# rajasekarv/vega

Measured on AMD Instinct MI355X. Metric: rows/sec (whole node) reduce_by_key i64→i64, 1e9 rows, 1/2/4/8 GPU, higher is better.
Workload: dtype int64; 1 GPU; C1: 1e9 (i64,i64) uniform keys in [0,2^63), reduce_by_key(sum), 256 partitions (BASELINE.json configs[1]); weak scaling: --rows per GPU; rows_per_gpu=1000000000, key_bits=63, nparts=256, distinct_keys_out=1000000000

## Files before the change

vega_amd/csrc/vega_kernels.hip:

```cpp

#include <hip/hip_runtime.h>
#include <cmath>
#include <cstdint>
#include <cstdio>
#include <cstring>
#include <mutex>
#include <string>
#include <unordered_map>
#include <vector>

#include "../../include/vega_common.h"
#include "vega_internal.h"

#define HIP_TRY(x)                                                              \
    do {                                                                        \
        hipError_t _e = (x);                                                    \
        if (_e != hipSuccess) return _e;                                        \
    } while (0)

namespace vega {

constexpr int BLOCK = 256;
constexpr int IPT = 16;
constexpr int TILE = BLOCK * IPT;
// ... 1324 lines not shown
        uint64_t g0;
        int m;
        bounds(tile, &g0, &m);
        const int a0 = (int)(t0 - g0), a1 = (int)(t1 - g0);
        if (threadIdx.x == 0) s_bad = 0;
#pragma unroll
        for (int q = 0; q < FIN_LPT; ++q) {
            int li = q * FIN_B + threadIdx.x;
            h[q] = (uint32_t)vega_hash_u64(r[q].x);
            if (li < m) s_row[li] = r[q];
            if (lane == 63) s_edge[q * (FIN_B / 64) + w] = h[q] >> 8;
        }
        __syncthreads();
        VEGA_PHASE_MARK(0)
        const uint32_t next = tile + gridDim.x;
        if (next < ntiles) fetch(next);
        const bool done = order_tile(g0, m, a0, a1);
        if (done) {
            const int lo = lo_out;
            uint32_t heads = 0;
            uint16_t si[FIN_FT / FIN_B], sp[FIN_FT / FIN_B];
#pragma unroll
            for (int q = 0; q < FIN_FT / FIN_B; ++q) {
                const int p = a0 + q * FIN_B + threadIdx.x;
                const int pc = p < a1 ? p : a1 - 1;
                si[q] = s_src[pc];
                sp[q] = s_src[pc > lo ? pc - 1 : pc];
            }
            ulonglong2 row[FIN_FT / FIN_B];
            uint64_t pkey[FIN_FT / FIN_B];
#pragma unroll
            for (int q = 0; q < FIN_FT / FIN_B; ++q) {
                row[q] = s_row[si[q]];
                pkey[q] = s_row[sp[q]].x;
            }
#pragma unroll
            for (int q = 0; q < FIN_FT / FIN_B; ++q) {
                const int p = a0 + q * FIN_B + threadIdx.x;
                if (p < a1) ((ulonglong2 *)out)[g0 + p] = row[q];
                const bool head = p < a1 && (p == lo || row[q].x != pkey[q]);
                heads += (uint32_t)__popcll(__ballot(head));
            }
            if (lane == 0) s_heads[w] = heads;
        }
        VEGA_PHASE_MARK(4)
        __syncthreads();
        if (done && threadIdx.x == 0) {
            uint32_t t = 0;
#pragma unroll
            for (int i = 0; i < FIN_B / 64; ++i) t += s_heads[i];
            fin_heads[tile] = t;
        }
        VEGA_PHASE_MARK(5)
        tile = next;
    }
    if (PROF && lane == 0)
        for (int i = 0; i < FIN_PHASES; ++i) atomicAdd(&phc[FIN_PHASE0 + i], pacc[i]);
#undef VEGA_PHASE_MARK
}

__global__ void k_unpack_rows(const uint64_t *pk, uint64_t n, uint64_t *k, uint64_t *v) {
    uint64_t stride = (uint64_t)gridDim.x * blockDim.x;
    for (uint64_t i = (uint64_t)blockIdx.x * blockDim.x + threadIdx.x; i < n; i += stride) {
        ulonglong2 r = ((const ulonglong2 *)pk)[i];
        k[i] = r.x;
        v[i] = r.y;
    }
}

hipError_t group_sort_u64(hipStream_t s, const uint64_t *in_k, const uint64_t *in_v,
                          uint64_t n, int force_hbytes, int *order_tag,
                          int want_packed, int *out_packed, Ws &ws,
                          const uint64_t **res_k, const uint64_t **res_v,
                          int route, int *route_taken, const uint32_t **fin_heads) {
    *res_k = in_k;
    *res_v = in_v;
    if (out_packed) *out_packed = 0;
    if (order_tag) *order_tag = 0;
    if (route_taken) *route_taken = 0;
    if (fin_heads) *fin_heads = nullptr;
    if (n <= 1) return hipSuccess;
    if (n >= (1ULL << 32)) return hipErrorNotSupported;
    uint32_t nb = nblocks_for(n);

    uint64_t *pA = (uint64_t *)ws.take(n * 16);
    uint64_t *pB = (uint64_t *)ws.take(n * 16);
    unsigned long long *desc = (unsigned long long *)ws.take((size_t)256 * nb * 8);
    uint32_t *gbase_d = (uint32_t *)ws.take(8 * 256 * 4);
    uint32_t *ticket = (uint32_t *)ws.take(256);
    uint32_t *h8 = (uint32_t *)ws.take(8 * 256 * 4);
    int *d_err = (int *)ws.take(256);
    int *d_abort = (int *)ws.take(256);
    unsigned long long *ff_d = (unsigned long long *)ws.take(
        ((size_t)((nb + OSW_GRP - 1) / OSW_GRP) +
         (size_t)((nb + OSW_SUP - 1) / OSW_SUP)) * 256 * 8);
    uint32_t *h32buf = (uint32_t *)ws.take(n * 4);
    unsigned long long *wl = (unsigned long long *)ws.take(CLEANUP_WL_CAP * 8);
    uint32_t *wl_count = (uint32_t *)ws.take(256);
    uint32_t *fh_d = (uint32_t *)ws.take(((size_t)2 * nb + 1) * 4);
    if (!pA || !pB || !desc || !gbase_d || !ticket || !h8 || !d_err || !d_abort ||
        !ff_d || !h32buf || !wl || !wl_count || !fh_d)
        return hipErrorOutOfMemory;
    HIP_TRY(hipMemsetAsync(d_abort, 0, 4, s));
    HIP_TRY(hipMemsetAsync(desc, 0, (size_t)nb * 256 * 8, s));
    int ptag_ctr = 0;
    const int strict = (force_hbytes != 0 || order_tag != nullptr) ? 1 : 0;

    static thread_local uint32_t hh[8 * 256];
    static thread_local uint32_t gb_host[8 * 256];
    bool pass_on[8] = {true, true, true, true, true, true, true, true};

    auto exact_hists = [&](bool hashsrc, int nbl, int *active) -> hipError_t {
        HIP_TRY(hipMemsetAsync(h8, 0, 8 * 256 * 4, s));
        {
            ProfScope ps(hashsrc ? "ghist" : "hist8", s);
            uint32_t gb = nb < 2048 ? nb : 2048;
            if (hashsrc && nbl == 4)
                hipLaunchKernelGGL((k_hist8t<true, 4>), dim3(gb), dim3(BLOCK), 0, s, in_k, n, h8);
            else if (hashsrc)
                hipLaunchKernelGGL((k_hist8t<true, 5>), dim3(gb), dim3(BLOCK), 0, s, in_k, n, h8);
            else
                hipLaunchKernelGGL((k_hist8t<false, 8>), dim3(gb), dim3(BLOCK), 0, s, in_k, n, h8);
            HIP_TRY(hipGetLastError());
        }
        HIP_TRY(hipMemcpyAsync(hh, h8, 8 * 256 * 4, hipMemcpyDeviceToHost, s));
        HIP_TRY(hipStreamSynchronize(s));
        *active = 0;
        for (int p = 0; p < 8; ++p) {
            int nz = 0;
            uint32_t running = 0;
            for (int d = 0; d < 256; ++d) {
                nz += hh[p * 256 + d] != 0;
                gb_host[p * 256 + d] = running;
                running += hh[p * 256 + d];
            }
            pass_on[p] = nz > 1;
            *active += pass_on[p];
        }
        return hipMemcpyAsync(gbase_d, gb_host, 8 * 256 * 4, hipMemcpyHostToDevice, s);
    };

    auto run_key_passes = [&](const uint64_t **rk, const uint64_t **rv) -> hipError_t {
        int plist[8], np = 0;
        for (int p = 0; p < 8; ++p)
            if (pass_on[p]) plist[np++] = p;
        if (np == 0) { *rk = in_k; *rv = in_v; return hipSuccess; }
        const uint64_t *cur = nullptr;
        for (int i = 0; i < np; ++i) {
            int p = plist[i];
            bool in_pk = i > 0, out_pk = i < np - 1;
            uint64_t *dbuf = ((i & 1) == 0) ? pA : pB;
            uint64_t *dk = dbuf;
            uint64_t *dv = out_pk ? nullptr : dbuf + n;
            RadixDigit df{8 * p};
            HIP_TRY(scatter_pass_osw(s, i == 0 ? in_k : cur, i == 0 ? in_v : nullptr,
                                     n, gbase_d + p * 256, desc, ticket,
                                     dk, dv, nullptr, d_abort, ff_d, ptag_ctr++, true, in_pk, out_pk, df, "radix_scatter"));
            cur = dk;
        }
        *rk = cur;
        *rv = cur + n;
        return hipSuccess;
    };

    int a_est = 8;
    bool samp_repeat = false;
    double bucket_rows = 0;
    HIP_TRY(sample_active_passes(s, in_k, n, ws, &a_est, &samp_repeat, &bucket_rows));

    const uint64_t *cur_k = in_k, *cur_v = in_v;
    if (a_est <= 5 && route == 0) {
        int active = 8;
        HIP_TRY(exact_hists(false, 8, &active));
        if (active <= 5) {
            HIP_TRY(run_key_passes(res_k, res_v));
            int ab = 0;
            HIP_TRY(hipMemcpyAsync(&ab, d_abort, 4, hipMemcpyDeviceToHost, s));
            HIP_TRY(hipStreamSynchronize(s));
            return ab ? hipErrorUnknown : hipSuccess;
        }
    }

    const int hbytes = force_hbytes ? force_hbytes : ((n <= (1ULL << 30)) ? 4 : 5);
    int active5 = 0;
    HIP_TRY(exact_hists(true, hbytes, &active5));
    const bool keep_pk = want_packed != 0;
    if (!strict && hbytes == 4 && keep_pk && route != 1 &&
        (route == 2 || (!samp_repeat && bucket_rows >= FIN_MIN_BUCKET_ROWS))) {
        for (int i = 1; i < 4; ++i) {
            uint64_t *dk = (i & 1) ? pA : pB;
            HashByteDigit df{8 * i};
            HIP_TRY(scatter_pass_osw(s, i == 1 ? in_k : cur_k, i == 1 ? in_v : nullptr,
                                     n, gbase_d + i * 256, desc, ticket, dk, nullptr, nullptr,
                                     d_abort, ff_d, ptag_ctr++, true, i > 1, true, df, "radix_scatter"));
            cur_k = dk;
        }
        HIP_TRY(hipMemsetAsync(d_err, 0, 4, s));
        {
            ProfScope ps("group_cleanup", s);
            ProfScope pk("bucket_finish", s);
            const uint32_t ntiles = (uint32_t)((n + FIN_FT - 1) / FIN_FT);
            unsigned long long *phc = phase_prof_buf();
            const dim3 grid(ntiles < FIN_GRID ? ntiles : FIN_GRID);
            if (phc)
                hipLaunchKernelGGL(k_bucket_finish<true>, grid, dim3(FIN_B), 0, s, cur_k, pB, n,
                                   d_err, fh_d, phc);
            else
                hipLaunchKernelGGL(k_bucket_finish<false>, grid, dim3(FIN_B), 0, s, cur_k, pB, n,
                                   d_err, fh_d, nullptr);
            HIP_TRY(hipGetLastError());
        }
        int fl[2] = {0, 0};
        HIP_TRY(hipMemcpyAsync(&fl[0], d_err, 4, hipMemcpyDeviceToHost, s));
        HIP_TRY(hipMemcpyAsync(&fl[1], d_abort, 4, hipMemcpyDeviceToHost, s));
        HIP_TRY(hipStreamSynchronize(s));
        if (fl[1]) return hipErrorUnknown;
        if (!fl[0]) {
            if (out_packed) *out_packed = 1;
            if (route_taken) *route_taken = 2;
            if (fin_heads) *fin_heads = fh_d;
            *res_k = pB;
            *res_v = nullptr;
            return hipSuccess;
        }
        cur_k = in_k;
        cur_v = in_v;
    }
    if (route_taken) *route_taken = 1;
    for (int i = 0; i < hbytes; ++i) {
        bool in_pk = i > 0, out_pk = keep_pk || (i < hbytes - 1);
        bool last = i == hbytes - 1;
        uint64_t *dbuf = ((i & 1) == 0) ? pA : pB;
        uint64_t *dk = dbuf;
        uint64_t *dv = out_pk ? nullptr : dbuf + n;
        HashByteDigit df{8 * i};
        HIP_TRY(scatter_pass_osw(s, i == 0 ? in_k : cur_k, i == 0 ? in_v : nullptr,
                                 n, gbase_d + i * 256, desc, ticket,
                                 dk, dv, last ? h32buf : nullptr,
                                 d_abort, ff_d, ptag_ctr++, true, in_pk, out_pk, df, "radix_scatter"));
        cur_k = dk;
        cur_v = out_pk ? nullptr : dk + n;
    }
    HIP_TRY(hipMemsetAsync(d_err, 0, 4, s));
    HIP_TRY(hipMemsetAsync(wl_count, 0, 4, s));
    {
        ProfScope ps("group_cleanup", s);
        uint32_t gb = nb < 2048 ? nb : 2048;
        hipLaunchKernelGGL(k_group_cleanup, dim3(gb), dim3(BLOCK), 0, s,
                           (uint64_t *)cur_k, (uint64_t *)cur_v, h32buf, n,
                           keep_pk ? 1 : 0, strict, d_err, wl, wl_count);
        HIP_TRY(hipGetLastError());
        hipLaunchKernelGGL(k_group_cleanup_long, dim3(512), dim3(BLOCK), 0, s,
                           cur_k, h32buf, n, keep_pk ? 1 : 0, strict, d_err, wl, wl_count);
        HIP_TRY(hipGetLastError());
    }
    int flags[2] = {0, 0};
    HIP_TRY(hipMemcpyAsync(&flags[0], d_err, 4, hipMemcpyDeviceToHost, s));
    HIP_TRY(hipMemcpyAsync(&flags[1], d_abort, 4, hipMemcpyDeviceToHost, s));
    HIP_TRY(hipStreamSynchronize(s));
    if (flags[1]) return hipErrorUnknown;
    int err = flags[0];
    if (err) {
        int active = 8;
        HIP_TRY(exact_hists(false, 8, &active));
        HIP_TRY(run_key_passes(&cur_k, &cur_v));
        int ab2 = 0;
        HIP_TRY(hipMemcpyAsync(&ab2, d_abort, 4, hipMemcpyDeviceToHost, s));
        HIP_TRY(hipStreamSynchronize(s));
        if (ab2) return hipErrorUnknown;
    } else if (keep_pk && out_packed) {
        *out_packed = 1;
    }
    if (order_tag && !err) *order_tag = (hbytes == 4) ? 4 : 0;
    *res_k = cur_k;
    *res_v = cur_v;
    return hipSuccess;
}


template <bool PK>
__global__ void k_head_count(const uint64_t *k, uint64_t n, uint32_t *hc) {
    __shared__ uint32_t wsum[BLOCK / 64];
    uint64_t tbase = (uint64_t)blockIdx.x * TILE;
    uint32_t c = 0;
#pragma unroll
    for (int j = 0; j < IPT; ++j) {
        uint64_t idx = tbase + (uint64_t)j * BLOCK + threadIdx.x;
        if (idx < n)
            c += (idx == 0) || (k[PK ? 2 * idx : idx] != k[PK ? 2 * (idx - 1) : idx - 1]);
    }
    for (int off = 32; off > 0; off >>= 1) c += __shfl_down(c, off);
    int lane = threadIdx.x & 63, w = threadIdx.x >> 6;
    if (lane == 0) wsum[w] = c;
    __syncthreads();
    if (threadIdx.x == 0) {
        uint32_t t = 0;
        for (int i = 0; i < BLOCK / 64; ++i) t += wsum[i];
        hc[blockIdx.x] = t;
    }
}

#define SEG_B 512
#define SEG_IPT 8
template <int OP, bool PK>
__global__ __launch_bounds__(SEG_B) void k_seg_emit(
    const uint64_t *__restrict__ k, const void *__restrict__ vv, uint64_t n,
    const uint32_t *__restrict__ head_base, uint32_t hstride,
    int64_t *__restrict__ out_k, void *__restrict__ out_vv,
    uint32_t *__restrict__ lead_seg, double *__restrict__ lead_part) {
    __shared__ uint32_t wsc[SEG_B / 64];
    constexpr bool NEED_V = (OP != 1);

    const int t = threadIdx.x, lane = t & 63, w = t >> 6;
    const uint64_t tbase = (uint64_t)blockIdx.x * TILE;
    const uint64_t *v = (const uint64_t *)vv;
    const uint64_t c0g = tbase + (uint64_t)t * SEG_IPT;

    uint64_t kk[SEG_IPT], sv[SEG_IPT];
    if (c0g + SEG_IPT <= n) {
        if (PK) {
            const ulonglong2 *rp = reinterpret_cast<const ulonglong2 *>(k) + c0g;
#pragma unroll
            for (int j = 0; j < SEG_IPT; ++j) {
                ulonglong2 r2 = rp[j];
                kk[j] = r2.x;
                sv[j] = r2.y;
            }
        } else {
            const ulonglong2 *kp = reinterpret_cast<const ulonglong2 *>(k + c0g);
            const ulonglong2 *vp = reinterpret_cast<const ulonglong2 *>(v + c0g);
#pragma unroll
            for (int j2 = 0; j2 < SEG_IPT / 2; ++j2) {
                ulonglong2 t2 = kp[j2];
                kk[2 * j2] = t2.x;
                kk[2 * j2 + 1] = t2.y;
                if (NEED_V) {
                    ulonglong2 u2 = vp[j2];
                    sv[2 * j2] = u2.x;
                    sv[2 * j2 + 1] = u2.y;
                }
            }
        }
    } else {
#pragma unroll
        for (int j = 0; j < SEG_IPT; ++j) {
            uint64_t gi = c0g + j;
            kk[j] = (gi < n) ? k[PK ? 2 * gi : gi] : ~0ULL;
            if (NEED_V || PK) sv[j] = (gi < n) ? (PK ? k[2 * gi + 1] : v[gi]) : 0;
        }
    }
    uint64_t prev = (c0g > 0 && c0g <= n) ? k[PK ? 2 * (c0g - 1) : c0g - 1] : 0;

    uint32_t cnt = 0;
#pragma unroll
    for (int j = 0; j < SEG_IPT; ++j) {
        uint64_t gi = c0g + j;
        if (gi < n) {
            uint64_t pk = (j > 0) ? kk[j - 1] : prev;
            cnt += (gi == 0) || (kk[j] != pk);
        }
    }
    uint32_t inc = cnt;
    for (int off = 1; off < 64; off <<= 1) {
        uint32_t u = __shfl_up(inc, off);
        if (lane >= off) inc += u;
    }
    if (lane == 63) wsc[w] = inc;
    __syncthreads();
    uint32_t excl = inc - cnt;
    for (int i = 0; i < w; ++i) excl += wsc[i];

    if (OP == 2) {
        uint64_t chunk_id = (uint64_t)blockIdx.x * SEG_B + t;
        int64_t sid = (int64_t)head_base[(size_t)blockIdx.x * hstride] + excl - 1;
        if (c0g >= n) {
            lead_seg[chunk_id] = 0xFFFFFFFFu;
            return;
        }
        int nvalid = (int)((n - c0g < SEG_IPT) ? (n - c0g) : SEG_IPT);
        int fh = -1;
        for (int j = 0; j < nvalid; ++j) {
            uint64_t pk2 = (j > 0) ? kk[j - 1] : prev;
            if (c0g + j == 0 || kk[j] != pk2) { fh = j; break; }
        }
        int le = (fh >= 0) ? fh : nvalid;
        if (le > 0) {
            double lead = 0.0;
            for (int j = 0; j < le; ++j) lead += __longlong_as_double((long long)sv[j]);
            lead_seg[chunk_id] = (uint32_t)sid;
            lead_part[chunk_id] = lead;
        } else {
            lead_seg[chunk_id] = 0xFFFFFFFFu;
        }
        if (fh >= 0) {
            double acc = 0.0;
            for (int j = fh; j < nvalid; ++j) {
                uint64_t pk2 = (j > 0) ? kk[j - 1] : prev;
                bool head = (c0g + j == 0) || (kk[j] != pk2);
                if (head) {
                    if (j > fh) ((double *)out_vv)[sid] = acc;
                    sid++;
                    out_k[sid] = (int64_t)kk[j];
                    acc = 0.0;
                }
                acc += __longlong_as_double((long long)sv[j]);
            }
            ((double *)out_vv)[sid] = acc;
        }
        return;
    }

    const uint64_t chunk_id = (uint64_t)blockIdx.x * SEG_B + t;
    if (c0g >= n) {
        lead_seg[chunk_id] = 0xFFFFFFFFu;
        return;
    }
    constexpr int64_t IDENT = (OP == 3) ? INT64_MAX : (OP == 4) ? INT64_MIN : 0;
    auto fold = [](int64_t a, uint64_t x) -> int64_t {
        if (OP == 0) return (int64_t)((uint64_t)a + x);
        if (OP == 1) return a + 1;
        if (OP == 3) return (int64_t)x < a ? (int64_t)x : a;
        return (int64_t)x > a ? (int64_t)x : a;
    };
    int64_t segid = (int64_t)head_base[(size_t)blockIdx.x * hstride] + excl - 1;
    if (cnt == SEG_IPT && c0g + SEG_IPT <= n) {
        int64_t s0 = segid + 1;
        int64_t *okp = (int64_t *)out_k + s0;
        uint64_t *ovp = (uint64_t *)out_vv + s0;
        if ((s0 & 1) == 0) {
            ulonglong2 *ok2 = (ulonglong2 *)okp;
            ulonglong2 *ov2 = (ulonglong2 *)ovp;
#pragma unroll
            for (int j = 0; j < SEG_IPT / 2; ++j) {
                ok2[j] = make_ulonglong2(kk[2 * j], kk[2 * j + 1]);
                if (OP == 1) ov2[j] = make_ulonglong2(1, 1);
                else ov2[j] = make_ulonglong2(sv[2 * j], sv[2 * j + 1]);
            }
        } else {
#pragma unroll
            for (int j = 0; j < SEG_IPT; ++j) {
                okp[j] = (int64_t)kk[j];
                ovp[j] = (OP == 1) ? 1ULL : sv[j];
            }
        }
        lead_seg[chunk_id] = 0xFFFFFFFFu;
        return;
    }
    const int64_t open_seg = segid;
    int64_t lead = IDENT, acc = IDENT;
    bool seen = false;
#pragma unroll
    for (int j = 0; j < SEG_IPT; ++j) {
        uint64_t gi = c0g + j;
        if (gi < n) {
            uint64_t pk = (j > 0) ? kk[j - 1] : prev;
            if (gi == 0 || kk[j] != pk) {
                if (seen) ((int64_t *)out_vv)[segid] = acc;
                segid++;
                out_k[segid] = (int64_t)kk[j];
                acc = IDENT;
                seen = true;
            }
            if (seen) acc = fold(acc, sv[j]);
            else lead = fold(lead, sv[j]);
        }
    }
    if (seen) ((int64_t *)out_vv)[segid] = acc;
    if (c0g != 0 && kk[0] == prev) {
        lead_seg[chunk_id] = (uint32_t)open_seg;
        ((int64_t *)lead_part)[chunk_id] = lead;
    } else {
        lead_seg[chunk_id] = 0xFFFFFFFFu;
    }
}

constexpr int SEG_FOLD_U = 4;
template <int OP>
__global__ __launch_bounds__(BLOCK) void k_seg_lead_fold(
    const uint32_t *__restrict__ lead_seg, const int64_t *__restrict__ lead_part,
    uint64_t nchunks, int64_t *__restrict__ out_v) {
    const int lane = threadIdx.x & 63;
    constexpr int U = SEG_FOLD_U;
    const uint64_t stride = (uint64_t)gridDim.x * BLOCK * U;
    for (uint64_t c0 = (uint64_t)blockIdx.x * BLOCK * U; c0 < nchunks; c0 += stride) {
        uint32_t sgs[U];
#pragma unroll
        for (int u = 0; u < U; ++u) {
            const uint64_t c = c0 + (uint64_t)u * BLOCK + threadIdx.x;
            sgs[u] = (c < nchunks) ? lead_seg[c] : 0xFFFFFFFFu;
        }
#pragma unroll
        for (int u = 0; u < U; ++u) {
            const uint64_t c = c0 + (uint64_t)u * BLOCK + threadIdx.x;
            const uint32_t sg = sgs[u];
            const bool have = sg != 0xFFFFFFFFu;
            if (!__any(have)) continue;
            int64_t acc = have ? lead_part[c] : 0;
            long long sid = have ? (long long)sg : -(long long)(lane + 2);
#pragma unroll
            for (int off = 1; off < 64; off <<= 1) {
                long long s2 = __shfl_up(sid, off);
                long long a2 = __shfl_up((long long)acc, off);
                if (lane >= off && s2 == sid) {
                    if (OP == 3) acc = (int64_t)a2 < acc ? (int64_t)a2 : acc;
                    else if (OP == 4) acc = (int64_t)a2 > acc ? (int64_t)a2 : acc;
                    else acc = (int64_t)((uint64_t)acc + (uint64_t)a2);
                }
            }
            long long snext = __shfl_down(sid, 1);
            if (have && (lane == 63 || snext != sid)) {
                if (OP == 0 || OP == 1) atomicAdd((unsigned long long *)(out_v + sg), (unsigned long long)acc);
                else if (OP == 3) atomicMin((long long *)(out_v + sg), (long long)acc);
                else atomicMax((long long *)(out_v + sg), (long long)acc);
            }
        }
    }
}

__global__ void k_f64_seg_combine(const uint32_t *lead_seg, const double *lead_part,
                                  uint64_t nchunks, double *out_v) {
    uint64_t stride = (uint64_t)gridDim.x * blockDim.x;
    for (uint64_t c = (uint64_t)blockIdx.x * blockDim.x + threadIdx.x; c < nchunks; c += stride) {
        uint32_t sg = lead_seg[c];
        if (sg == 0xFFFFFFFFu) continue;
        if (c > 0 && lead_seg[c - 1] == sg) continue;
        double acc = 0.0;
        uint64_t x = c;
        while (x < nchunks && lead_seg[x] == sg) { acc += lead_part[x]; ++x; }
        out_v[sg] += acc;
    }
}

static_assert(TILE == 2 * FIN_FT, "two finish tiles per segmented-reduce tile");
static hipError_t seg_head_bases(hipStream_t s, const uint64_t *k, uint64_t n, bool packed,
                                 const uint32_t *fin_heads, Ws &ws, const uint32_t **hc_out,
                                 uint32_t *hstride, const uint32_t **total_d) {
    const uint32_t nb = nblocks_for(n);
    ProfScope ps("head_count", s);
    uint32_t *hc;
    uint64_t nent;
    if (fin_heads) {
        hc = const_cast<uint32_t *>(fin_heads);
        nent = (uint64_t)2 * nb;
        *hstride = 2;
        const uint64_t nfin = (n + FIN_FT - 1) / FIN_FT;
        HIP_TRY(hipMemsetAsync(hc + nfin, 0, (size_t)(nent + 1 - nfin) * 4, s));
    } else {
        hc = (uint32_t *)ws.take(((size_t)nb + 1) * 4);
        if (!hc) return hipErrorOutOfMemory;
        nent = nb;
        *hstride = 1;
        if (packed)
            hipLaunchKernelGGL((k_head_count<true>), dim3(nb), dim3(BLOCK), 0, s, k, n, hc);
        else
            hipLaunchKernelGGL((k_head_count<false>), dim3(nb), dim3(BLOCK), 0, s, k, n, hc);
        HIP_TRY(hipGetLastError());
        HIP_TRY(hipMemsetAsync(hc + nb, 0, 4, s));
    }
    {
        Ws w2 = ws;
        HIP_TRY(scan_u32_excl(s, hc, nent + 1, w2));
    }
    *hc_out = hc;
    *total_d = hc + nent;
    return hipSuccess;
}

hipError_t seg_reduce(hipStream_t s, const uint64_t *k, const void *v, uint64_t n,
                      int op, uint64_t *out_k, void *out_v, uint64_t *h_nout, Ws &ws,
                      bool packed, const uint32_t *fin_heads) {
    if (n == 0) { *h_nout = 0; return hipSuccess; }
    if (n >= (1ULL << 32)) return hipErrorNotSupported;
    if (op < 0 || op > 4) return hipErrorInvalidValue;
    uint32_t nb = nblocks_for(n);
    uint64_t nchunks = (uint64_t)nb * SEG_B;
    uint32_t *lead_seg = (uint32_t *)ws.take(nchunks * 4);
    double *lead_part = (double *)ws.take(nchunks * 8);
    if (!lead_seg || !lead_part) return hipErrorOutOfMemory;
    const uint32_t *hc, *total_d;
    uint32_t hstride;
    HIP_TRY(seg_head_bases(s, k, n, packed, fin_heads, ws, &hc, &hstride, &total_d));
    uint32_t total = 0;
    HIP_TRY(hipMemcpyAsync(&total, total_d, 4, hipMemcpyDeviceToHost, s));
    {
        ProfScope ps("seg_emit", s);
        size_t sh = 0;
#define SEG_LAUNCH(OPN, PKB) hipLaunchKernelGGL((k_seg_emit<OPN, PKB>), dim3(nb), dim3(SEG_B), sh, s, k, v, n, hc, hstride, (int64_t *)out_k, out_v, lead_seg, lead_part)
        switch (op * 2 + (packed ? 1 : 0)) {
        case 0: SEG_LAUNCH(0, false); break;
        case 1: SEG_LAUNCH(0, true); break;
        case 2: SEG_LAUNCH(1, false); break;
        case 3: SEG_LAUNCH(1, true); break;
        case 4: SEG_LAUNCH(2, false); break;
        case 5: SEG_LAUNCH(2, true); break;
        case 6: SEG_LAUNCH(3, false); break;
        case 7: SEG_LAUNCH(3, true); break;
        case 8: SEG_LAUNCH(4, false); break;
        case 9: SEG_LAUNCH(4, true); break;
        default: return hipErrorInvalidValue;
        }
#undef SEG_LAUNCH
        HIP_TRY(hipGetLastError());
    }
    if (op == 2) {
        ProfScope ps("f64_combine", s);
        uint32_t gb = nb < 2048 ? nb : 2048;
        hipLaunchKernelGGL(k_f64_seg_combine, dim3(gb), dim3(BLOCK), 0, s,
                           lead_seg, lead_part, nchunks, (double *)out_v);
        HIP_TRY(hipGetLastError());
    } else {
        ProfScope ps("seg_fold", s);
        const uint64_t per = (uint64_t)BLOCK * SEG_FOLD_U;
        const uint64_t rounds = (nchunks + per - 1) / per;
        uint32_t gb = (uint32_t)(rounds < 4096 ? rounds : 4096);
        const int64_t *lp = (const int64_t *)lead_part;
        switch (op) {
        case 0:
        case 1:
            hipLaunchKernelGGL((k_seg_lead_fold<0>), dim3(gb), dim3(BLOCK), 0, s, lead_seg, lp,
                               nchunks, (int64_t *)out_v);
            break;
        case 3:
            hipLaunchKernelGGL((k_seg_lead_fold<3>), dim3(gb), dim3(BLOCK), 0, s, lead_seg, lp,
                               nchunks, (int64_t *)out_v);
            break;
        default:
            hipLaunchKernelGGL((k_seg_lead_fold<4>), dim3(gb), dim3(BLOCK), 0, s, lead_seg, lp,
                               nchunks, (int64_t *)out_v);
            break;
        }
        HIP_TRY(hipGetLastError());
    }
    HIP_TRY(hipStreamSynchronize(s));
    *h_nout = total;
    return hipSuccess;
}

hipError_t group_sort_reduce(hipStream_t s, const uint64_t *in_k, const uint64_t *in_v,
                             uint64_t n, int op, uint64_t *out_k, void *out_v,
                             uint64_t *h_nout, Ws &ws) {
    if (n == 0) { *h_nout = 0; return hipSuccess; }
    const uint64_t *sk, *sv;
    int pk = 0;
    const uint32_t *fh = nullptr;
    hipError_t e = group_sort_u64(s, in_k, in_v, n, 0, nullptr, 1, &pk, ws, &sk, &sv, 0,
                                  nullptr, &fh);
    if (e != hipSuccess) return e;
    return seg_reduce(s, sk, sv, n, op, out_k, out_v, h_nout, ws, pk != 0, fh);
}

hipError_t group_rows(hipStream_t s, const uint64_t *in_k, const uint64_t *in_v, uint64_t n,
                      int route, uint64_t *out_k, uint64_t *out_v, Ws &ws, int *route_taken) {
    if (route_taken) *route_taken = 0;
    if (n == 0) return hipSuccess;
    const uint64_t *sk, *sv;
    int pk = 0;
    HIP_TRY(group_sort_u64(s, in_k, in_v, n, 0, nullptr, 1, &pk, ws, &sk, &sv, route, route_taken));
    if (pk) {
        uint32_t nb = nblocks_for(n);
        hipLaunchKernelGGL(k_unpack_rows, dim3(nb < 2048 ? nb : 2048), dim3(BLOCK), 0, s,
                           sk, n, out_k, out_v);
        return hipGetLastError();
    }
    HIP_TRY(hipMemcpyAsync(out_k, sk, n * 8, hipMemcpyDeviceToDevice, s));
    return hipMemcpyAsync(out_v, sv, n * 8, hipMemcpyDeviceToDevice, s);
}


struct StatsAcc {
    int64_t cnt, mn, mx;
    uint64_t sum;
    __device__ __forceinline__ void reset() { cnt = 0; sum = 0; mn = INT64_MAX; mx = INT64_MIN; }
    __device__ __forceinline__ void add(uint64_t v) {
        int64_t x = (int64_t)v;
        cnt += 1;
        sum += v;
        mn = x < mn ? x : mn;
        mx = x > mx ? x : mx;
    }
};

template <bool PK>
__global__ __launch_bounds__(SEG_B) void k_seg_stats(
    const uint64_t *__restrict__ k, const uint64_t *__restrict__ v, uint64_t n,
    const uint32_t *__restrict__ head_base, uint32_t hstride,
    int64_t *__restrict__ out_k,
    int64_t *__restrict__ out_count, int64_t *__restrict__ out_sum,
    int64_t *__restrict__ out_min, int64_t *__restrict__ out_max) {
    __shared__ uint32_t wsc[SEG_B / 64];

    const int t = threadIdx.x, lane = t & 63, w = t >> 6;
    const uint64_t tbase = (uint64_t)blockIdx.x * TILE;
    const uint64_t c0g = tbase + (uint64_t)t * SEG_IPT;

    uint64_t kk[SEG_IPT], sv[SEG_IPT];
    if (c0g + SEG_IPT <= n) {
        if (PK) {
            const ulonglong2 *rp = reinterpret_cast<const ulonglong2 *>(k) + c0g;
#pragma unroll
            for (int j = 0; j < SEG_IPT; ++j) {
                ulonglong2 r2 = rp[j];
                kk[j] = r2.x;
                sv[j] = r2.y;
            }
        } else {
            const ulonglong2 *kp = reinterpret_cast<const ulonglong2 *>(k + c0g);
            const ulonglong2 *vp = reinterpret_cast<const ulonglong2 *>(v + c0g);
#pragma unroll
            for (int j2 = 0; j2 < SEG_IPT / 2; ++j2) {
                ulonglong2 t2 = kp[j2];
                ulonglong2 u2 = vp[j2];
                kk[2 * j2] = t2.x;
                kk[2 * j2 + 1] = t2.y;
                sv[2 * j2] = u2.x;
                sv[2 * j2 + 1] = u2.y;
            }
        }
    } else {
#pragma unroll
        for (int j = 0; j < SEG_IPT; ++j) {
            uint64_t gi = c0g + j;
            kk[j] = (gi < n) ? k[PK ? 2 * gi : gi] : ~0ULL;
            sv[j] = (gi < n) ? (PK ? k[2 * gi + 1] : v[gi]) : 0;
        }
    }
    uint64_t prev = (c0g > 0 && c0g <= n) ? k[PK ? 2 * (c0g - 1) : c0g - 1] : 0;

// ... 1787 lines not shown
```

Baseline: 22.27 billion rows/s.

## Coalesce segment-emit loads per wavefront and stage through LDS transpose

k_seg_emit now loads each wavefront's 512-element span with lane-strided coalesced vector loads instead of per-thread contiguous chunks. Heads are counted via ballot/popcount with shuffle carries rather than a shuffle scan. A fast path writes all-distinct wave spans directly with coalesced stores. Otherwise data is transposed through a swizzled LDS stage buffer back to the per-thread blocked layout. This adds 32KB of shared memory per block, which may lower occupancy, plus extra wave-level syncs on the slow path.

```diff
diff --git a/vega_amd/csrc/vega_kernels.hip b/vega_amd/csrc/vega_kernels.hip
--- a/vega_amd/csrc/vega_kernels.hip
+++ b/vega_amd/csrc/vega_kernels.hip
@@ -1650,6 +1650,20 @@
 
 #define SEG_B 512
 #define SEG_IPT 8
+#define SEG_SPAN (64 * SEG_IPT)
+
+__device__ __forceinline__ void seg_stage_sync() {
+    __builtin_amdgcn_fence(__ATOMIC_RELEASE, "wavefront");
+    __builtin_amdgcn_wave_barrier();
+    __builtin_amdgcn_fence(__ATOMIC_ACQUIRE, "wavefront");
+}
+
+__device__ __forceinline__ uint64_t seg_lane63(uint64_t x) {
+    uint32_t lo = (uint32_t)__builtin_amdgcn_readlane((int)(uint32_t)x, 63);
+    uint32_t hi = (uint32_t)__builtin_amdgcn_readlane((int)(uint32_t)(x >> 32), 63);
+    return ((uint64_t)hi << 32) | lo;
+}
+
 template <int OP, bool PK>
 __global__ __launch_bounds__(SEG_B) void k_seg_emit(
     const uint64_t *__restrict__ k, const void *__restrict__ vv, uint64_t n,
@@ -1657,70 +1671,160 @@
     int64_t *__restrict__ out_k, void *__restrict__ out_vv,
     uint32_t *__restrict__ lead_seg, double *__restrict__ lead_part) {
     __shared__ uint32_t wsc[SEG_B / 64];
+    __shared__ __attribute__((aligned(16))) uint64_t stage[SEG_B / 64][SEG_SPAN];
     constexpr bool NEED_V = (OP != 1);
 
     const int t = threadIdx.x, lane = t & 63, w = t >> 6;
     const uint64_t tbase = (uint64_t)blockIdx.x * TILE;
     const uint64_t *v = (const uint64_t *)vv;
-    const uint64_t c0g = tbase + (uint64_t)t * SEG_IPT;
-
+    const uint64_t wbase = tbase + (uint64_t)w * SEG_SPAN;
+    const bool full = wbase + SEG_SPAN <= n;
+    const uint64_t chunk_id = (uint64_t)blockIdx.x * SEG_B + t;
+
+    auto srow = [&](int i) -> uint32_t {
+        return PK ? (uint32_t)(i * 64 + lane) : (uint32_t)((i >> 1) * 128 + 2 * lane + (i & 1));
+    };
+    uint64_t rk[SEG_IPT], rv[SEG_IPT], hm[SEG_IPT];
+    uint64_t gprev = 0;
+    uint32_t wheads = 0;
+    if (wbase < n) {
+        if (full) {
+            if (PK) {
+                const ulonglong2 *rp = reinterpret_cast<const ulonglong2 *>(k) + wbase + lane;
+#pragma unroll
+                for (int i = 0; i < SEG_IPT; ++i) {
+                    ulonglong2 r2 = rp[i * 64];
+                    rk[i] = r2.x;
+                    rv[i] = r2.y;
+                }
+            } else {
+                const ulonglong2 *kp = reinterpret_cast<const ulonglong2 *>(k + wbase) + lane;
+                const ulonglong2 *vp = reinterpret_cast<const ulonglong2 *>(v + wbase) + lane;
+#pragma unroll
+                for (int q = 0; q < SEG_IPT / 2; ++q) {
+                    ulonglong2 t2 = kp[q * 64];
+                    rk[2 * q] = t2.x;
+                    rk[2 * q + 1] = t2.y;
+                    if (NEED_V) {
+                        ulonglong2 u2 = vp[q * 64];
+                        rv[2 * q] = u2.x;
+                        rv[2 * q + 1] = u2.y;
+                    }
+                }
+            }
+        } else {
+#pragma unroll
+            for (int i = 0; i < SEG_IPT; ++i) {
+                uint64_t gi = wbase + srow(i);
+                rk[i] = (gi < n) ? k[PK ? 2 * gi : gi] : ~0ULL;
+                if (NEED_V || PK) rv[i] = (gi < n) ? (PK ? k[2 * gi + 1] : v[gi]) : 0;
+            }
+        }
+        if (wbase > 0) gprev = k[PK ? 2 * (wbase - 1) : wbase - 1];
+
+        uint64_t carry = gprev;
+#pragma unroll
+        for (int i = 0; i < SEG_IPT; ++i) {
+            uint64_t pk;
+            if (PK || !(i & 1)) {
+                const uint64_t last = PK ? rk[i] : rk[i + 1];
+                pk = __shfl_up(last, 1);
+                if (lane == 0) pk = carry;
+                carry = seg_lane63(last);
+            } else {
+                pk = rk[i - 1];
+            }
+            uint64_t gi = wbase + srow(i);
+            hm[i] = __ballot(gi < n && (gi == 0 || rk[i] != pk));
+            wheads += (uint32_t)__popcll(hm[i]);
+        }
+    }
+    if (lane == 0) wsc[w] = wheads;
+    __syncthreads();
+    if (wbase >= n) {
+        lead_seg[chunk_id] = 0xFFFFFFFFu;
+        return;
+    }
+    uint32_t wexcl = 0;
+    for (int i = 0; i < w; ++i) wexcl += wsc[i];
+    const int64_t tile_base = (int64_t)head_base[(size_t)blockIdx.x * hstride];
+
+    if (full && wheads == SEG_SPAN) {
+        int64_t *okp = out_k + tile_base + wexcl;
+        uint64_t *ovp = (uint64_t *)out_vv + tile_base + wexcl;
+        auto outv = [&](int i) -> uint64_t {
+            if (OP == 1) return 1ULL;
+            if (OP == 2) {
+                double acc = 0.0;
+                acc += __longlong_as_double((long long)rv[i]);
+                return (uint64_t)__double_as_longlong(acc);
+            }
+            return rv[i];
+        };
+        if (!PK && ((tile_base + wexcl) & 1) == 0) {
+            ulonglong2 *ok2 = (ulonglong2 *)okp + lane;
+            ulonglong2 *ov2 = (ulonglong2 *)ovp + lane;
+#pragma unroll
+            for (int q = 0; q < SEG_IPT / 2; ++q) {
+                ok2[q * 64] = make_ulonglong2(rk[2 * q], rk[2 * q + 1]);
+                ov2[q * 64] = make_ulonglong2(outv(2 * q), outv(2 * q + 1));
+            }
+        } else {
+#pragma unroll
+            for (int i = 0; i < SEG_IPT; ++i) {
+                okp[srow(i)] = (int64_t)rk[i];
+                ovp[srow(i)] = outv(i);
+            }
+        }
+        lead_seg[chunk_id] = 0xFFFFFFFFu;
+        return;
+    }
+
+    uint64_t *st = stage[w];
+    auto swz = [](int s) -> int { return s ^ ((s >> 4) & 3); };
+    auto hand_over = [&](const uint64_t(&src)[SEG_IPT], uint64_t(&dst)[SEG_IPT]) {
+        if (PK) {
+#pragma unroll
+            for (int i = 0; i < SEG_IPT; ++i)
+                st[2 * swz(i * 32 + (lane >> 1)) + (lane & 1)] = src[i];
+        } else {
+#pragma unroll
+            for (int q = 0; q < SEG_IPT / 2; ++q)
+                *reinterpret_cast<ulonglong2 *>(st + 2 * swz(q * 64 + lane)) =
+                    make_ulonglong2(src[2 * q], src[2 * q + 1]);
+        }
+        seg_stage_sync();
+#pragma unroll
+        for (int j2 = 0; j2 < SEG_IPT / 2; ++j2) {
+            ulonglong2 t2 = *reinterpret_cast<const ulonglong2 *>(st + 2 * swz(lane * (SEG_IPT / 2) + j2));
+            dst[2 * j2] = t2.x;
+            dst[2 * j2 + 1] = t2.y;
+        }
+        seg_stage_sync();
+    };
     uint64_t kk[SEG_IPT], sv[SEG_IPT];
-    if (c0g + SEG_IPT <= n) {
-        if (PK) {
-            const ulonglong2 *rp = reinterpret_cast<const ulonglong2 *>(k) + c0g;
-#pragma unroll
-            for (int j = 0; j < SEG_IPT; ++j) {
-                ulonglong2 r2 = rp[j];
-                kk[j] = r2.x;
-                sv[j] = r2.y;
-            }
-        } else {
-            const ulonglong2 *kp = reinterpret_cast<const ulonglong2 *>(k + c0g);
-            const ulonglong2 *vp = reinterpret_cast<const ulonglong2 *>(v + c0g);
-#pragma unroll
-            for (int j2 = 0; j2 < SEG_IPT / 2; ++j2) {
-                ulonglong2 t2 = kp[j2];
-                kk[2 * j2] = t2.x;
-                kk[2 * j2 + 1] = t2.y;
-                if (NEED_V) {
-                    ulonglong2 u2 = vp[j2];
-                    sv[2 * j2] = u2.x;
-                    sv[2 * j2 + 1] = u2.y;
-                }
-            }
-        }
-    } else {
-#pragma unroll
-        for (int j = 0; j < SEG_IPT; ++j) {
-            uint64_t gi = c0g + j;
-            kk[j] = (gi < n) ? k[PK ? 2 * gi : gi] : ~0ULL;
-            if (NEED_V || PK) sv[j] = (gi < n) ? (PK ? k[2 * gi + 1] : v[gi]) : 0;
-        }
-    }
-    uint64_t prev = (c0g > 0 && c0g <= n) ? k[PK ? 2 * (c0g - 1) : c0g - 1] : 0;
-
-    uint32_t cnt = 0;
-#pragma unroll
-    for (int j = 0; j < SEG_IPT; ++j) {
-        uint64_t gi = c0g + j;
-        if (gi < n) {
-            uint64_t pk = (j > 0) ? kk[j - 1] : prev;
-            cnt += (gi == 0) || (kk[j] != pk);
-        }
-    }
-    uint32_t inc = cnt;
-    for (int off = 1; off < 64; off <<= 1) {
-        uint32_t u = __shfl_up(inc, off);
-        if (lane >= off) inc += u;
-    }
-    if (lane == 63) wsc[w] = inc;
-    __syncthreads();
-    uint32_t excl = inc - cnt;
-    for (int i = 0; i < w; ++i) excl += wsc[i];
+    hand_over(rk, kk);
+    if (NEED_V || PK) hand_over(rv, sv);
+    const uint64_t c0g = wbase + (uint64_t)lane * SEG_IPT;
+    uint64_t prev = __shfl_up(kk[SEG_IPT - 1], 1);
+    if (lane == 0) prev = gprev;
+
+    constexpr int GW = PK ? SEG_IPT : SEG_IPT / 2;
+    const int grp = lane / (64 / GW), gsh = (lane % (64 / GW)) * GW;
+    uint32_t cnt = 0, excl = wexcl;
+#pragma unroll
+    for (int i = 0; i < SEG_IPT; ++i) {
+        const int g = PK ? i : (i >> 1);
+        if (g < grp) {
+            excl += (uint32_t)__popcll(hm[i]);
+        } else if (g == grp) {
+            cnt += (uint32_t)__popcll((hm[i] >> gsh) & ((1ULL << GW) - 1));
+            excl += (uint32_t)__popcll(hm[i] & ((1ULL << gsh) - 1));
+        }
+    }
 
     if (OP == 2) {
-        uint64_t chunk_id = (uint64_t)blockIdx.x * SEG_B + t;
-        int64_t sid = (int64_t)head_base[(size_t)blockIdx.x * hstride] + excl - 1;
+        int64_t sid = tile_base + excl - 1;
         if (c0g >= n) {
             lead_seg[chunk_id] = 0xFFFFFFFFu;
             return;
@@ -1758,7 +1862,6 @@
         return;
     }
 
-    const uint64_t chunk_id = (uint64_t)blockIdx.x * SEG_B + t;
     if (c0g >= n) {
         lead_seg[chunk_id] = 0xFFFFFFFFu;
         return;
@@ -1770,7 +1873,7 @@
         if (OP == 3) return (int64_t)x < a ? (int64_t)x : a;
         return (int64_t)x > a ? (int64_t)x : a;
     };
-    int64_t segid = (int64_t)head_base[(size_t)blockIdx.x * hstride] + excl - 1;
+    int64_t segid = tile_base + excl - 1;
     if (cnt == SEG_IPT && c0g + SEG_IPT <= n) {
         int64_t s0 = segid + 1;
         int64_t *okp = (int64_t *)out_k + s0;
```

Measured after the change: 23.31 billion rows/s (median of 6 runs). 1.05x the previous value.
